# CartoonSegmentation/CartoonSegmentation

Measured on AMD Instinct MI355X. Metric: frames/sec at 1024x1024 (seg+depth+warp), higher is better.
Workload: dtype f32; 1 GPU; seg(RTMDet-Ins-L det640 + maskhead + ISNet refine@720, 2 instances) + LeReS depth@640 + 1 warp, frame 1024x1024; frames_per_gpu_step=8, global_batch=8, weights=closed-form synthetic (no checkpoints offline), precision=fp32 exact (v_mfma_f32_32x32x2_f32)

## Files before the change

cartoonsegmentation_amd/csrc/csm_convcfg.h:

```cpp
#pragma once
#include "csm_conv.h"
#include <span>
#include <utility>

#ifndef CSM_ILV
#define CSM_ILV 1
#endif

#ifdef CSM_CONV_ABLATE
#define CSM_DBG(a) ((a).dbg)
#else
#define CSM_DBG(a) 0
#endif

namespace csmconv {

constexpr int kLdsLd = 36;

typedef float f32x4v __attribute__((ext_vector_type(4)));

enum { CFG_128x128_4w = 0, CFG_128x64 = 1, CFG_64x64 = 2, CFG_128x128_8w = 3, CFG_128x32 = 4, CFG_64x16 = 5,
       CFG_D64x64 = 6, CFG_D128x64 = 7, CFG_D128x128 = 8, CFG_D128x128_8w = 9, CFG_D256x128_8w = 10, CFG_D64x128 = 11, CFG_D128x32 = 12,
       CFG_NARROW = 13,
       CFG_D96x128 = 14, CFG_D160x128 = 15, CFG_D224x128 = 16, CFG_D192x128 = 17,
       CFG_P64x64 = 18, CFG_P128x64 = 19, CFG_P64x128 = 20, CFG_P128x128 = 21, CFG_P256x128 = 22, CFG_P128x32 = 23,
       CFG_P64x64_w8 = 24, CFG_P128x128_w8 = 25, CFG_P128x32_w8 = 26, CFG_P128x128_8w = 27,
       CFG_D64x64_s3 = 28, CFG_D128x64_s3 = 29, CFG_D64x128_s3 = 30, CFG_D128x128_s3 = 31, CFG_D128x128_8w_s3 = 32,
       CFG_D256x128_8w_s3 = 33, CFG_D256x64 = 34, CFG_D256x64_s3 = 35, CFG_P256x64 = 36, CFG_D64x64_s4 = 37,
       CFG_Q64x64 = 38, CFG_Q128x64 = 39, CFG_Q64x128 = 40, CFG_Q128x128_8w = 41, CFG_Q128x32 = 42,
       CFG_R128x32 = 43, CFG_R64x64 = 44, CFG_R128x64 = 45, CFG_R128x32_w8 = 46, CFG_R128x128_8w = 47, CFG_R64x128 = 48, CFG_R64x64_w8 = 49,
       CFG_R128x128_8w_o4 = 50,
       CFG_W256x32 = 51, CFG_W256x64 = 52,
       CFG_COUNT = 53 };

enum ConvFamily {
    FAM_MFMA,
    FAM_DMA,
    FAM_PATCH,
    FAM_DMA_P,
    FAM_PATCH_P,
    FAM_WS,
    FAM_NARROW,
    FAM_COUNT
};
constexpr bool fam_uses_dma(int f) { return f != FAM_MFMA && f != FAM_NARROW; }
constexpr bool fam_needs_patch(int f) { return f == FAM_PATCH || f == FAM_PATCH_P || f == FAM_WS; }
constexpr bool fam_persistent(int f) { return f == FAM_DMA_P || f == FAM_PATCH_P || f == FAM_WS; }

struct ConvCfg {
    int id;
    const char *name;
    int family;
    int bn;
    int (*launch)(const ConvArgs &, hipStream_t);
};
std::span<const ConvCfg> conv_cfgs_mfma();
std::span<const ConvCfg> conv_cfgs_dma();
std::span<const ConvCfg> conv_cfgs_patch();
std::span<const ConvCfg> conv_cfgs_narrow();

bool dma_eligible(const ConvArgs &a);
bool patch_eligible(const ConvArgs &a);
bool narrow_eligible(const ConvArgs &a);
constexpr int kWsPatchBytes = 2 * (((16 + 2) * (16 + 2) + 7) / 8 + 1) * 1024;
bool ws_fits(const ConvArgs &a, int BN);

extern int g_ngroup_enable;
int choose_ngroup(const ConvArgs &a, int BN);
int launch_reduce(const ConvArgs &a, hipStream_t st);

int launch_conv_stem(const ConvArgs &a, hipStream_t st);
int launch_netop(const csm_op &op, int i, const View &in, const View &in1, const View &out, const float *weights, hipStream_t st);

}
```

cartoonsegmentation_amd/csrc/netops.hip:

```cpp
#include "csm_convcfg.h"

using namespace csmconv;

namespace {

__global__ __launch_bounds__(256) void k_conv_stem(ConvArgs a) {
    constexpr int BM = 64, BN = 64;
    __shared__ __attribute__((aligned(16))) float lds[(BM + BN) * kLdsLd];
    const int tid = threadIdx.x, lane = tid & 63, wave = tid >> 6;
    const int wm = wave >> 1, wn = wave & 1, li = lane & 31, lh = lane >> 5;
    int mt, ntile, zz;
    block_to_tile(mt, ntile, zz);
    const int m0 = mt * BM, n0 = ntile * BN;
    const int ho = a.out.h, wo = a.out.w, ntaps = a.kh * a.kw, nck = (ntaps + 7) >> 3;
    const int j = tid & 7;
    const float *rowp[2]; int iy0[2], ix0[2]; bool rv[2];
#pragma unroll
    for (int it = 0; it < 2; ++it) {
        int m = m0 + (tid >> 3) + 32 * it;
        rv[it] = m < a.M;
        int mm = rv[it] ? m : 0;
        int n = mm / (ho * wo), rem = mm - n * ho * wo;
        int oy = rem / wo, ox = rem - oy * wo;
        iy0[it] = oy * a.stride - a.pad; ix0[it] = ox * a.stride - a.pad;
// ... 319 lines not shown
    int b = blockIdx.x;
    const int tx = b % tiles_x; b /= tiles_x;
    const int ty = b % tiles_y, n = b / tiles_y;
    const int c0 = blockIdx.y * 32;
    const int oy0 = ty * TH, ox0 = tx * TW, iy0 = oy0 - a.pad, ix0 = ox0 - a.pad;
    for (int i = tid; i < taps * 32; i += 256) wl[i] = a.w[(int64_t)(i >> 5) * a.out.c + c0 + (i & 31)];
    const int total = rh * rw * 8;
    for (int i0 = tid; i0 < total; i0 += 256 * 4) {
        float4 v[4];
#pragma unroll
        for (int u = 0; u < 4; ++u) {
            int i = i0 + u * 256;
            v[u] = make_float4(0.f, 0.f, 0.f, 0.f);
            if (i < total) {
                int c4 = i & 7, pix = i >> 3;
                int ry = pix / rw, rx = pix - ry * rw;
                int iy = iy0 + ry, ix = ix0 + rx;
                if (iy >= 0 && iy < a.in.h && ix >= 0 && ix < a.in.w)
                    v[u] = *reinterpret_cast<const float4 *>(a.in.p + ((int64_t)(n * a.in.h + iy) * a.in.w + ix) * a.in.ld + c0 + c4 * 4);
            }
        }
#pragma unroll
        for (int u = 0; u < 4; ++u) {
            int i = i0 + u * 256;
            if (i < total) *reinterpret_cast<float4 *>(xl + (i >> 3) * 32 + (i & 7) * 4) = v[u];
        }
    }
    __syncthreads();
    const int c4 = tid & 7, p0 = tid >> 3;
    const float4 bias = a.bias ? *reinterpret_cast<const float4 *>(a.bias + c0 + c4 * 4) : make_float4(0.f, 0.f, 0.f, 0.f);
    const float4 sl = a.slope ? *reinterpret_cast<const float4 *>(a.slope + c0 + c4 * 4) : make_float4(0.f, 0.f, 0.f, 0.f);
    float4 acc[4];
#pragma unroll
    for (int j = 0; j < 4; ++j) acc[j] = bias;
    for (int kh = 0; kh < a.kh; ++kh)
        for (int kw = 0; kw < a.kw; ++kw) {
            const float4 w = *reinterpret_cast<const float4 *>(wl + (kh * a.kw + kw) * 32 + c4 * 4);
#pragma unroll
            for (int j = 0; j < 4; ++j) {
                const int pix = p0 + 32 * j, py = pix >> 4, px = pix & 15;
                const float4 x = *reinterpret_cast<const float4 *>(xl + ((py + kh) * rw + px + kw) * 32 + c4 * 4);
                acc[j].x = fmaf(x.x, w.x, acc[j].x); acc[j].y = fmaf(x.y, w.y, acc[j].y);
                acc[j].z = fmaf(x.z, w.z, acc[j].z); acc[j].w = fmaf(x.w, w.w, acc[j].w);
            }
        }
#pragma unroll
    for (int j = 0; j < 4; ++j) {
        const int pix = p0 + 32 * j, oy = oy0 + (pix >> 4), ox = ox0 + (pix & 15);
        if (oy >= a.out.h || ox >= a.out.w) continue;
        float4 v = acc[j];
        v.x = apply_act(v.x, a.act, sl.x); v.y = apply_act(v.y, a.act, sl.y);
        v.z = apply_act(v.z, a.act, sl.z); v.w = apply_act(v.w, a.act, sl.w);
        *reinterpret_cast<float4 *>(a.out.p + ((int64_t)(n * a.out.h + oy) * a.out.w + ox) * a.out.ld + c0 + c4 * 4) = v;
    }
}

__global__ __launch_bounds__(256) void k_maxpool(View in, View out, int k, int stride, int pad) {
    const int c4n = out.c >> 2;
    int64_t idx = (int64_t)blockIdx.x * 256 + threadIdx.x;
    int64_t total = (int64_t)out.n * out.h * out.w * c4n;
    if (idx >= total) return;
    int c = (int)(idx % c4n) * 4; int64_t pix = idx / c4n;
    int ox = (int)(pix % out.w); int64_t t = pix / out.w; int oy = (int)(t % out.h); int n = (int)(t / out.h);
    float4 m = make_float4(-INFINITY, -INFINITY, -INFINITY, -INFINITY);
    for (int ky = 0; ky < k; ++ky) {
        int iy = oy * stride - pad + ky;
        if (iy < 0 || iy >= in.h) continue;
        for (int kx = 0; kx < k; ++kx) {
            int ix = ox * stride - pad + kx;
            if (ix < 0 || ix >= in.w) continue;
            float4 x = *reinterpret_cast<const float4 *>(in.p + ((int64_t)(n * in.h + iy) * in.w + ix) * in.ld + c);
            m.x = fmaxf(m.x, x.x); m.y = fmaxf(m.y, x.y); m.z = fmaxf(m.z, x.z); m.w = fmaxf(m.w, x.w);
        }
    }
    *reinterpret_cast<float4 *>(out.p + pix * out.ld + c) = m;
}

__device__ __forceinline__ void src_index(int dst, int in_size, int out_size, float scale, bool align, int &i0, int &i1,
                                          float &l0, float &l1) {
    if (in_size == out_size) { i0 = i1 = dst; l0 = 1.0f; l1 = 0.0f; return; }
    float real;
    if (align) real = scale * (float)dst;
    else { real = scale * ((float)dst + 0.5f) - 0.5f; if (real < 0.0f) real = 0.0f; }
    i0 = min((int)real, in_size - 1);
    i1 = i0 + (i0 < in_size - 1 ? 1 : 0);
    l1 = fminf(fmaxf(real - (float)i0, 0.0f), 1.0f);
    l0 = 1.0f - l1;
}

template <int VEC>
__global__ __launch_bounds__(256) void k_bilinear(View in, View out, int align, float sh, float sw, int act, const float *__restrict__ slope) {
    const int cv = out.c / VEC;
    int64_t idx = (int64_t)blockIdx.x * 256 + threadIdx.x;
    int64_t total = (int64_t)out.n * out.h * out.w * cv;
    if (idx >= total) return;
    int c = (int)(idx % cv) * VEC; int64_t pix = idx / cv;
    int ox = (int)(pix % out.w); int64_t t = pix / out.w; int oy = (int)(t % out.h); int n = (int)(t / out.h);
    int y0, y1, x0, x1; float hl0, hl1, wl0, wl1;
    src_index(oy, in.h, out.h, sh, align != 0, y0, y1, hl0, hl1);
    src_index(ox, in.w, out.w, sw, align != 0, x0, x1, wl0, wl1);
    const float *P = in.p + (int64_t)n * in.h * in.w * in.ld + c;
    const float *a00 = P + ((int64_t)y0 * in.w + x0) * in.ld, *a01 = P + ((int64_t)y0 * in.w + x1) * in.ld;
    const float *a10 = P + ((int64_t)y1 * in.w + x0) * in.ld, *a11 = P + ((int64_t)y1 * in.w + x1) * in.ld;
    float *O = out.p + pix * out.ld + c;
    if (VEC == 4) {
        float4 p00 = *reinterpret_cast<const float4 *>(a00), p01 = *reinterpret_cast<const float4 *>(a01);
// ... 138 lines not shown
    for (int k = 0; k < K; ++k) {
        const float y = (lb[k] + (float)k * lx + (float)(K - 1 - k) * lo) / t;
        const float e = csm_expf(y - mx);
        den += e; num += e * c[k];
    }
    out.p[pix * out.ld] = num / den;
}

__global__ __launch_bounds__(256) void k_gavgpool(View in, View out) {
    __shared__ float part[256];
    int c = blockIdx.x, n = blockIdx.y;
    int hw = in.h * in.w;
    const float *P = in.p + (int64_t)n * hw * in.ld + c;
    float s = 0.0f;
    for (int i = threadIdx.x; i < hw; i += 256) s += P[(int64_t)i * in.ld];
    part[threadIdx.x] = s;
    __syncthreads();
    for (int st = 128; st >= 1; st >>= 1) {
        if ((int)threadIdx.x < st) part[threadIdx.x] += part[threadIdx.x + st];
        __syncthreads();
    }
    if (threadIdx.x == 0) out.p[(int64_t)n * out.ld + c] = part[0] / (float)hw;
}

__global__ __launch_bounds__(256) void k_gavgpool32(View in, View out) {
    __shared__ float part[256][33];
    const int c0 = blockIdx.x * 32, n = blockIdx.y, t = threadIdx.x;
    const int hw = in.h * in.w;
    const float *P = in.p + (int64_t)n * hw * in.ld + c0;
    float s[32];
#pragma unroll
    for (int c = 0; c < 32; ++c) s[c] = 0.0f;
    for (int i = t; i < hw; i += 256) {
        const float4 *q = reinterpret_cast<const float4 *>(P + (int64_t)i * in.ld);
#pragma unroll
        for (int c4 = 0; c4 < 8; ++c4) {
            float4 v = q[c4];
            s[4 * c4] += v.x; s[4 * c4 + 1] += v.y; s[4 * c4 + 2] += v.z; s[4 * c4 + 3] += v.w;
        }
    }
#pragma unroll
    for (int c = 0; c < 32; ++c) part[t][c] = s[c];
    __syncthreads();
    for (int st = 128; st >= 1; st >>= 1) {
        for (int i = t; i < st * 32; i += 256) {
            int r = i >> 5, c = i & 31;
            part[r][c] += part[r + st][c];
        }
        __syncthreads();
    }
    if (t < 32) out.p[(int64_t)n * out.ld + c0 + t] = part[0][t] / (float)hw;
}

__global__ __launch_bounds__(256) void k_nchw_to_nhwc(const float *__restrict__ src, int csrc, View out) {
    int64_t idx = (int64_t)blockIdx.x * 256 + threadIdx.x;
    int64_t total = (int64_t)out.n * out.h * out.w * out.c;
    if (idx >= total) return;
    int c = (int)(idx % out.c); int64_t pix = idx / out.c;
    int64_t hw = (int64_t)out.h * out.w; int64_t n = pix / hw, p = pix - n * hw;
    out.p[pix * out.ld + c] = c < csrc ? src[(n * csrc + c) * hw + p] : 0.0f;
}

__global__ __launch_bounds__(256) void k_nhwc_to_nchw(View in, float *__restrict__ dst) {
    int64_t idx = (int64_t)blockIdx.x * 256 + threadIdx.x;
    int64_t hw = (int64_t)in.h * in.w;
    int64_t total = (int64_t)in.n * in.c * hw;
    if (idx >= total) return;
    int64_t p = idx % hw; int64_t t = idx / hw; int c = (int)(t % in.c); int64_t n = t / in.c;
    dst[idx] = in.p[(n * hw + p) * in.ld + c];
}

constexpr int kTrPix = 64;
__global__ __launch_bounds__(256) void k_nchw_to_nhwc_tile(const float *__restrict__ src, int csrc, View out) {
    extern __shared__ float tr[];
    const int64_t hw = (int64_t)out.h * out.w;
    const int64_t tiles = (hw + kTrPix - 1) / kTrPix;
    const int64_t n = blockIdx.x / tiles, p0 = (blockIdx.x - n * tiles) * kTrPix;
    const int C = out.c;
    for (int i = threadIdx.x; i < C * kTrPix; i += 256) {
        const int c = i >> 6, p = i & 63;
        tr[c * (kTrPix + 1) + p] = (c < csrc && p0 + p < hw) ? src[(n * csrc + c) * hw + p0 + p] : 0.0f;
    }
    __syncthreads();
    for (int i = threadIdx.x; i < C * kTrPix; i += 256) {
        const int p = i / C, c = i - p * C;
        if (p0 + p < hw) out.p[(n * hw + p0 + p) * out.ld + c] = tr[c * (kTrPix + 1) + p];
    }
}
__global__ __launch_bounds__(256) void k_nhwc_to_nchw_tile(View in, float *__restrict__ dst) {
    extern __shared__ float tr[];
    const int64_t hw = (int64_t)in.h * in.w;
    const int64_t tiles = (hw + kTrPix - 1) / kTrPix;
    const int64_t n = blockIdx.x / tiles, p0 = (blockIdx.x - n * tiles) * kTrPix;
    const int C = in.c;
    for (int i = threadIdx.x; i < C * kTrPix; i += 256) {
        const int p = i / C, c = i - p * C;
        tr[c * (kTrPix + 1) + p] = p0 + p < hw ? in.p[(n * hw + p0 + p) * in.ld + c] : 0.0f;
    }
    __syncthreads();
    for (int i = threadIdx.x; i < C * kTrPix; i += 256) {
        const int c = i >> 6, p = i & 63;
        if (p0 + p < hw) dst[(n * C + c) * hw + p0 + p] = tr[c * (kTrPix + 1) + p];
    }
}

inline unsigned blocks_for(int64_t total) { return (unsigned)((total + 255) / 256); }

constexpr ConvCfg kRows[] = {{CFG_NARROW, "NARROW", FAM_NARROW, 4, &launch_narrow}};

}

std::span<const ConvCfg> csmconv::conv_cfgs_narrow() { return kRows; }

bool csmconv::narrow_eligible(const ConvArgs &a) {
    return a.cout_g <= 4 && a.groups == 1 && a.ksplit == 1 && !(a.cin_g & 3) && !(a.in.ld & 3) && narrow_lds(a, 4, nullptr, nullptr) != 0;
}

int csmconv::launch_reduce(const ConvArgs &a, hipStream_t st) {
    k_splitk_reduce<<<(unsigned)(((int64_t)a.M * a.cout_g + 255) / 256), 256, 0, st>>>(a);
    return csm::check_launch("k_splitk_reduce");
}

int csmconv::launch_conv_stem(const ConvArgs &a, hipStream_t st) {
    dim3 grid((a.M + 63) / 64, (a.cout_g + 63) / 64, 1);
    k_conv_stem<<<grid, 256, 0, st>>>(a);
    return csm::check_launch("k_conv_stem");
}

int csmconv::launch_netop(const csm_op &op, int i, const View &in, const View &in1, const View &out, const float *weights, hipStream_t st) {
    switch (op.kind) {
        case CSM_OP_DWCONV: {
            if ((in.ld & 3) || (out.ld & 3) || (out.c & 3)) { csm::set_error("op %d: dwconv needs c%%4==0", i); return CSM_ERR_ARG; }
            DwArgs a{in, out, weights + op.w_off, op.b_off >= 0 ? weights + op.b_off : nullptr,
                     op.aux_off >= 0 ? weights + op.aux_off : nullptr, op.kh, op.kw, op.stride, op.pad, op.dil, op.act};
            size_t lds = ((size_t)op.kh * op.kw * 32 + (size_t)(8 + op.kh - 1) * (16 + op.kw - 1) * 32) * 4;
            if (op.stride == 1 && op.dil == 1 && !(out.c & 31) && lds <= 64 * 1024 && out.h == in.h + 2 * op.pad - op.kh + 1) {
                int tiles_x = (out.w + 15) / 16, tiles_y = (out.h + 7) / 8;
                k_dwconv_lds<<<dim3((unsigned)(tiles_x * tiles_y * out.n), (unsigned)(out.c / 32)), 256, lds, st>>>(a, tiles_x, tiles_y);
            } else
                k_dwconv<<<blocks_for((int64_t)out.n * out.h * out.w * (out.c >> 2)), 256, 0, st>>>(a);
            break;
        }
        case CSM_OP_MAXPOOL:
            if ((in.ld & 3) || (out.ld & 3) || (out.c & 3)) { csm::set_error("op %d: maxpool needs c%%4==0", i); return CSM_ERR_ARG; }
            k_maxpool<<<blocks_for((int64_t)out.n * out.h * out.w * (out.c >> 2)), 256, 0, st>>>(in, out, op.kh, op.stride, op.pad);
            break;
        case CSM_OP_BILINEAR: {
            bool align = op.flags & 1;
            float sh, sw;
            if (align) { sh = out.h > 1 ? (float)(in.h - 1) / (float)(out.h - 1) : 0.0f; sw = out.w > 1 ? (float)(in.w - 1) / (float)(out.w - 1) : 0.0f; }
            else { sh = (float)in.h / (float)out.h; sw = (float)in.w / (float)out.w; }
            bool vec = !(out.c & 3) && !(in.ld & 3) && !(out.ld & 3) && !(((uintptr_t)in.p | (uintptr_t)out.p) & 15);
            const float *bsl = op.aux_off >= 0 ? weights + op.aux_off : nullptr;
            if (vec && out.h <= 65535 && out.n <= 65535 && (int64_t)out.w * (out.c >> 2) < (1ll << 30)) {
                unsigned mul, shr;
                set_fast_div((unsigned)(out.c >> 2), mul, shr);
                k_bilinear_rows<<<dim3(blocks_for((int64_t)out.w * (out.c >> 2)), (unsigned)out.h, (unsigned)out.n), 256, 0, st>>>(in, out, align ? 1 : 0, sh, sw, op.act, bsl, mul, shr);
            } else if (vec) k_bilinear<4><<<blocks_for((int64_t)out.n * out.h * out.w * (out.c >> 2)), 256, 0, st>>>(in, out, align ? 1 : 0, sh, sw, op.act, bsl);
            else k_bilinear<1><<<blocks_for((int64_t)out.n * out.h * out.w * out.c), 256, 0, st>>>(in, out, align ? 1 : 0, sh, sw, op.act, bsl);
            break;
        }
        case CSM_OP_NEAREST:
            if ((in.ld & 3) || (out.ld & 3) || (out.c & 3)) { csm::set_error("op %d: nearest needs c%%4==0", i); return CSM_ERR_ARG; }
            k_nearest<<<blocks_for((int64_t)out.n * out.h * out.w * (out.c >> 2)), 256, 0, st>>>(in, out);
            break;
        case CSM_OP_ADD:
            if (in.h < out.h || in.w < out.w || in.h > out.h + 1 || in.w > out.w + 1 || in1.h != out.h || in1.w != out.w) {
                csm::set_error("op %d: add: the first operand may exceed the output by at most one row / column", i); return CSM_ERR_ARG;
            }
            if (in.h == out.h && in.w == out.w && eltwise4_ok(in, &in1, out, nullptr))
                k_eltwise4<<<blocks_for((int64_t)out.n * out.h * out.w * (out.c >> 2)), 256, 0, st>>>(in, in1, out, op.act, 1, nullptr);
            else
                k_eltwise<<<blocks_for((int64_t)out.n * out.h * out.w * out.c), 256, 0, st>>>(in, in1, out, op.act,
                                                                                            (in.h != out.h || in.w != out.w) ? 3 : 1, nullptr);
            break;
        case CSM_OP_SCALE:
            k_eltwise<<<blocks_for((int64_t)out.n * out.h * out.w * out.c), 256, 0, st>>>(in, in1, out, op.act, 2, nullptr);
            break;
        case CSM_OP_ACT:
        case CSM_OP_COPY:
            if (eltwise4_ok(in, nullptr, out, op.aux_off >= 0 ? weights + op.aux_off : nullptr))
                k_eltwise4<<<blocks_for((int64_t)out.n * out.h * out.w * (out.c >> 2)), 256, 0, st>>>(in, in1, out, op.kind == CSM_OP_ACT ? op.act : 0, 0,
                                                                                                    op.aux_off >= 0 ? weights + op.aux_off : nullptr);
            else
                k_eltwise<<<blocks_for((int64_t)out.n * out.h * out.w * out.c), 256, 0, st>>>(in, in1, out, op.kind == CSM_OP_ACT ? op.act : 0, 0,
                                                                                              op.aux_off >= 0 ? weights + op.aux_off : nullptr);
            break;
        case CSM_OP_GAVGPOOL:
            if (!(in.c & 31) && !(in.ld & 3) && !(((uintptr_t)in.p) & 15)) k_gavgpool32<<<dim3(in.c / 32, in.n), 256, 0, st>>>(in, out);
            else k_gavgpool<<<dim3(in.c, in.n), 256, 0, st>>>(in, out);
            break;
        case CSM_OP_ATTRACTOR:
            if (op.aux_off < 0 || in.n != in1.n || in.h != in1.h || in.w != in1.w) { csm::set_error("op %d: attractor operands", i); return CSM_ERR_ARG; }
            k_attractor<<<blocks_for((int64_t)out.n * out.h * out.w * out.c), 256, 0, st>>>(in, in1, out, weights + op.aux_off, op.flags);
            break;
        case CSM_OP_LOGBINOM:
            if (op.aux_off < 0 || in.c < 4 || in1.c > 256) { csm::set_error("op %d: logbinom operands", i); return CSM_ERR_ARG; }
            k_logbinom<<<blocks_for((int64_t)out.n * out.h * out.w), 256, 0, st>>>(in, in1, out, weights + op.aux_off);
            break;
        case CSM_OP_NCHW_TO_NHWC:
            if (out.c >= 8 && out.c <= 240)
                k_nchw_to_nhwc_tile<<<(unsigned)(out.n * (((int64_t)out.h * out.w + kTrPix - 1) / kTrPix)), 256,
                                      sizeof(float) * (size_t)out.c * (kTrPix + 1), st>>>(in.p, in.c, out);
            else
                k_nchw_to_nhwc<<<blocks_for((int64_t)out.n * out.h * out.w * out.c), 256, 0, st>>>(in.p, in.c, out);
            break;
        case CSM_OP_NHWC_TO_NCHW:
            if (in.c >= 8 && in.c <= 240)
                k_nhwc_to_nchw_tile<<<(unsigned)(in.n * (((int64_t)in.h * in.w + kTrPix - 1) / kTrPix)), 256,
                                      sizeof(float) * (size_t)in.c * (kTrPix + 1), st>>>(in, out.p);
            else
                k_nhwc_to_nchw<<<blocks_for((int64_t)in.n * in.h * in.w * in.c), 256, 0, st>>>(in, out.p);
            break;
        default:
            csm::set_error("op %d: unknown kind %d", i, op.kind);
            return CSM_ERR_ARG;
    }
    return CSM_OK;
}
```

cartoonsegmentation_amd/csrc/nets.hip:

```cpp
#include "csm_common.h"
#include "csm_convcfg.h"
#include "csm_tokens.h"
#include <array>
#include <cstdio>
#include <cstdlib>
#include <cstring>
#include <map>
#include <mutex>
#include <vector>
#include <algorithm>
#include <utility>

using namespace csmconv;

int csmconv::g_ngroup_enable = 1;

static const ConvCfg &cfg_row(int id) {
    static const ConvCfg *table[CFG_COUNT];
    static const bool checked = [] {
        for (const std::span<const ConvCfg> rows : {conv_cfgs_mfma(), conv_cfgs_dma(), conv_cfgs_patch(), conv_cfgs_narrow()})
            for (const ConvCfg &r : rows) {
                if (r.id < 0 || r.id >= CFG_COUNT || table[r.id]) { fprintf(stderr, "csm355: conv tile configuration %d (%s) is out of range or defined twice\n", r.id, r.name); abort(); }
                table[r.id] = &r;
            }
// ... 118 lines not shown
                if (op.flags & CSM_CONV_FLAG_GROUPED) {
                    if (!grouped_eligible(a)) { csm::set_error("op %d: grouped-conv flag on an ineligible convolution (3x3 / stride 1 / pad 1 / cin_g == cout_g in {8, 16, 32} / channels %% 32 / ksplit 1)", i); return CSM_ERR_ARG; }
                    rc = launch_conv_grouped(a, st);
                    if (rc) return rc;
                    break;
                }
                if (op.flags & 2) {
                    if (op.groups != 1 || op.cin_g != 4 || a.ksplit != 1) { csm::set_error("op %d: stem flag needs groups 1, cin 4, ksplit 1", i); return CSM_ERR_ARG; }
                    rc = launch_conv_stem(a, st);
                    if (rc) return rc;
                    break;
                }
                const int tcfg = op.tile & (kTileSerial - 1);
                a.split = (op.tile & kTileSplit) != 0 && g_force_cfg < 0;
                const bool tuned = tcfg > 0 && tcfg <= CFG_COUNT && g_force_cfg < 0;
                a.serial = a.ksplit > 1 && (g_force_serial >= 0 ? g_force_serial != 0 : tuned ? (op.tile & kTileSerial) != 0
                                            : (int64_t)((a.M + 63) / 64) * ((op.cout_g + 63) / 64) >= 512);
                int cfg = tuned ? tcfg - 1 : choose_cfg(a, op.cout_g);
                rc = cfg_row(resolve_cfg(cfg, a)).launch(a, st);
                if (rc) return rc;
                break;
            }
            case CSM_OP_LAYERNORM: {
                if (op.w_off < 0 || op.b_off < 0 || op.aux_off < 0 || in.c != out.c) { csm::set_error("op %d: layernorm operands", i); return CSM_ERR_ARG; }
                rc = csm::launch_layernorm(in.p, in.ld, out.p, out.ld, (int64_t)in.n * in.h * in.w, in.c, weights + op.w_off, weights + op.b_off,
                                           weights + op.aux_off , st);
                if (rc) return rc;
                break;
            }
            case CSM_OP_ATTENTION: {
                const int heads = op.groups, d = op.cin_g;
                if (heads < 1 || in.c != 3 * heads * d || out.c != heads * d || in.w != 1 || out.h != in.h) { csm::set_error("op %d: attention operands", i); return CSM_ERR_ARG; }
                rc = csm::launch_attention(in.p, in.ld, out.p, out.ld, in.n, in.h, heads, d, op.aux_off >= 0 ? weights + op.aux_off : nullptr, op.kh, op.kw, st);
                if (rc) return rc;
                break;
            }
            case CSM_OP_TOKENS: {
                const int mode = op.flags;
                const int np = mode == 0 ? in.h * in.w : out.h * out.w;
                const bool ok = mode == 0 ? (out.h == np + 1 && out.w == 1 && out.c == in.c && op.aux_off >= 0)
                                          : (in.h == np + 1 && in.w == 1 && out.c == (mode == 1 ? 2 : 1) * in.c);
                if (!ok || in.n != out.n) { csm::set_error("op %d: tokens operands (mode %d)", i, mode); return CSM_ERR_ARG; }
                rc = csm::launch_tokens(mode, in.p, in.ld, out.p, out.ld, in.n, np, in.c, op.aux_off >= 0 ? weights + op.aux_off : nullptr, st);
                if (rc) return rc;
                break;
            }
            case CSM_OP_DEPTH_TO_SPACE: {
                const int k = op.stride;
                if (k < 1 || out.h != in.h * k || out.w != in.w * k || in.c != k * k * out.c) { csm::set_error("op %d: depth_to_space operands", i); return CSM_ERR_ARG; }
                rc = csm::launch_depth_to_space(in.p, in.ld, out.p, out.ld, in.n, in.h, in.w, k, out.c, st);
                if (rc) return rc;
                break;
            }
            default:
                rc = launch_netop(op, i, in, in1, out, weights, st);
                if (rc) return rc;
                break;
        }
        rc = csm::check_launch("program op");
        if (rc) { csm::set_error("op %d (kind %d) launch failed", i, op.kind); return rc; }
        if (ev) CSM_HIP(hipEventRecord(ev[i + 1], st));
    }
    return CSM_OK;
}

extern "C" int csm_run_program(const csm_op *ops, int n_ops, const csm_tensor_desc *tensors, int n_tensors,
                               const float *weights, float *workspace, void *const *ext, int n_ext, void *stream) {
    CSM_REQUIRE(ops && tensors && n_ops >= 0 && n_tensors > 0);
    return run_ops(ops, n_ops, tensors, n_tensors, weights, workspace, ext, n_ext, (hipStream_t)stream, nullptr);
}

struct EventSet {
    std::vector<hipEvent_t> ev;
    bool ok = true;
    explicit EventSet(size_t n) {
        ev.reserve(n);
        for (size_t i = 0; i < n; ++i) {
            hipEvent_t e;
            hipError_t r = hipEventCreate(&e);
            if (r != hipSuccess) { csm::set_error("hipEventCreate: %s", hipGetErrorString(r)); ok = false; return; }
            ev.push_back(e);
        }
    }
    ~EventSet() { for (auto e : ev) (void)hipEventDestroy(e); }
    EventSet(const EventSet &) = delete;
    EventSet &operator=(const EventSet &) = delete;
};

extern "C" int csm_run_program_profile(const csm_op *ops, int n_ops, const csm_tensor_desc *tensors, int n_tensors,
                                       const float *weights, float *workspace, void *const *ext, int n_ext, void *stream,
                                       float *op_ms) {
    CSM_REQUIRE(ops && tensors && op_ms && n_ops >= 0 && n_tensors > 0);
    hipStream_t st = (hipStream_t)stream;
    EventSet evs(n_ops + 1);
    if (!evs.ok) return CSM_ERR_HIP;
    int rc = run_ops(ops, n_ops, tensors, n_tensors, weights, workspace, ext, n_ext, st, evs.ev.data());
    if (rc == CSM_OK) {
        hipError_t e = hipStreamSynchronize(st);
        if (e != hipSuccess) { csm::set_error("profile sync: %s", hipGetErrorString(e)); rc = CSM_ERR_HIP; }
        else for (int i = 0; i < n_ops; ++i) (void)hipEventElapsedTime(&op_ms[i], evs.ev[i], evs.ev[i + 1]);
    }
    return rc;
}

static std::map<std::array<int, 16>, int> g_tile_cache;
static std::mutex g_tile_mutex;

extern "C" int csm_conv_autotune(csm_op *ops, int n_ops, const csm_tensor_desc *tensors, int n_tensors, const float *weights,
                                 float *workspace, void *const *ext, int n_ext, void *stream, int reps) {
    CSM_REQUIRE(ops && tensors && n_ops >= 0 && n_tensors > 0);
// ... 83 lines not shown
            if (timed[k].first < best) { best = timed[k].first; best_cfg = timed[k].second; }
        if (rc) break;
        op.tile = best_cfg >= 0 ? best_cfg + 1 : 0;
        { std::lock_guard<std::mutex> lk(g_tile_mutex); g_tile_cache[key] = op.tile; }
        ++tuned;
    }
    return rc == CSM_OK ? tuned : -rc;
}

extern "C" int csm_conv_tile_cache_save(const char *path) {
    CSM_REQUIRE(path);
    FILE *f = fopen(path, "w");
    if (!f) { csm::set_error("cannot write %s", path); return CSM_ERR_ARG; }
    std::lock_guard<std::mutex> lk(g_tile_mutex);
    for (const auto &kv : g_tile_cache) {
        for (int v : kv.first) fprintf(f, "%d ", v);
        fprintf(f, "%d\n", kv.second);
    }
    fclose(f);
    return CSM_OK;
}

extern "C" int csm_conv_tile_cache_load(const char *path) {
    CSM_REQUIRE(path);
    FILE *f = fopen(path, "r");
    if (!f) return 0;
    int n = 0;
    for (;;) {
        std::array<int, 16> key; int tile = 0; bool ok = true;
        for (int &v : key) ok = ok && fscanf(f, "%d", &v) == 1;
        if (!ok || fscanf(f, "%d", &tile) != 1) break;
        if (tile >= 0 && (tile & (kTileSerial - 1)) <= CFG_COUNT && tile < 2 * kTileSplit) { std::lock_guard<std::mutex> lk(g_tile_mutex); g_tile_cache[key] = tile; ++n; }
    }
    fclose(f);
    return n;
}

extern "C" int csm_debug_force_conv_cfg(int cfg) {
    if (cfg >= 0) { g_force_cfg = cfg & 0xff; g_dbg = cfg >> 8; } else { g_force_cfg = -1; g_dbg = 0; }
    return CSM_OK;
}

extern "C" int csm_debug_conv_tuner_options(int options) {
    g_tune_split = options & 1;
    g_ngroup_enable = (options & 2) ? 0 : 1;
    return CSM_OK;
}

extern "C" int csm_debug_force_splitk_serial(int mode) {
    g_force_serial = mode < 0 ? -1 : (mode ? 1 : 0);
    return CSM_OK;
}

extern "C" int csm_debug_conv_cfg_count(void) { return CFG_COUNT; }

extern "C" int csm_debug_conv_cfg_info(int cfg, csm_conv_cfg_desc *info) {
    CSM_REQUIRE(info);
    if (cfg < 0 || cfg >= CFG_COUNT) { csm::set_error("conv tile configuration %d out of range (0 .. %d)", cfg, CFG_COUNT - 1); return CSM_ERR_ARG; }
    static const char *const fam_names[FAM_COUNT] = {"MFMA", "DMA", "PATCH", "DMA_P", "PATCH_P", "WS", "NARROW"};
    const ConvCfg &r = cfg_row(cfg);
    info->id = r.id; info->bn = r.bn; info->name = r.name; info->family = fam_names[r.family];
    info->tune_pos = -1;
    for (size_t k = 0; k < sizeof(kTuneOrder) / sizeof(int); ++k)
        if (kTuneOrder[k] == cfg) info->tune_pos = (int)k;
    return CSM_OK;
}

extern "C" int csm_debug_conv_resolve_cfg(int cfg, const csm_op *op, const csm_tensor_desc *in_desc, const csm_tensor_desc *out_desc) {
    if (!op || !in_desc || !out_desc || cfg < 0 || cfg >= CFG_COUNT) { csm::set_error("conv_resolve_cfg: bad argument"); return -CSM_ERR_ARG; }
    return resolve_cfg(cfg, conv_args(*op, view_at(nullptr, *in_desc), view_at(nullptr, *out_desc), View{}, nullptr));
}
```

cartoonsegmentation_amd/program.py:

```python
import ctypes
import os

import numpy as np

OP_CONV, OP_DWCONV, OP_MAXPOOL, OP_BILINEAR, OP_NEAREST, OP_ADD, OP_GAVGPOOL, OP_SCALE = 1, 2, 3, 4, 5, 6, 7, 8
OP_NCHW_TO_NHWC, OP_NHWC_TO_NCHW, OP_ACT, OP_COPY, OP_ATTRACTOR, OP_LOGBINOM = 9, 10, 11, 12, 13, 14
OP_LAYERNORM, OP_ATTENTION, OP_TOKENS, OP_DEPTH_TO_SPACE = 15, 16, 17, 18
ACT = {None: 0, 'none': 0, 'relu': 1, 'silu': 2, 'prelu': 3, 'hsigmoid': 4, 'sigmoid': 5, 'softplus': 6, 'gelu': 7}


class CsmTensorDesc(ctypes.Structure):
    _fields_ = [("offset", ctypes.c_int64), ("ext", ctypes.c_int32), ("n", ctypes.c_int32), ("h", ctypes.c_int32),
                ("w", ctypes.c_int32), ("c", ctypes.c_int32), ("ld", ctypes.c_int32)]


class CsmOp(ctypes.Structure):
    _fields_ = [("kind", ctypes.c_int32), ("in0", ctypes.c_int32), ("in1", ctypes.c_int32), ("out", ctypes.c_int32),
                ("kh", ctypes.c_int32), ("kw", ctypes.c_int32), ("stride", ctypes.c_int32), ("pad", ctypes.c_int32),
                ("dil", ctypes.c_int32), ("groups", ctypes.c_int32), ("cin_g", ctypes.c_int32),
                ("cout_g", ctypes.c_int32), ("act", ctypes.c_int32), ("res_mode", ctypes.c_int32),
                ("w_off", ctypes.c_int64), ("b_off", ctypes.c_int64), ("aux_off", ctypes.c_int64),
                ("flags", ctypes.c_int32), ("ksplit", ctypes.c_int32), ("scratch", ctypes.c_int32),
                ("tile", ctypes.c_int32)]

# ... 388 lines not shown
        w_h, w_n = self._w(gamma, gamma)
        b_h, b_n = self._w(beta, beta)
        a_h, a_n = self._w(np.array([eps, 0, 0, 0], np.float32), np.array([eps, 0, 0, 0], np.float32))
        return self._emit(OP_LAYERNORM, x, None, out, w_off=w_h, b_off=b_h, aux_off=a_h, nat=dict(w_off=w_n, b_off=b_n, aux_off=a_n))

    def attention(self, qkv, heads, grid=None, rel_table=None):
        d = qkv.c // (3 * heads)
        assert qkv.w == 1 and qkv.c == 3 * heads * d and d in (32, 64, 128), (qkv.shape, heads)
        out = self.buffer(qkv.n, qkv.h, 1, heads * d)
        a_h = a_n = -1
        gh, gw = grid if grid is not None else (0, 0)
        if rel_table is not None:
            rel_table = np.asarray(rel_table, np.float32)
            assert rel_table.shape == ((2 * gh - 1) * (2 * gw - 1) + 3, heads) and qkv.h == gh * gw + 1, (rel_table.shape, grid, qkv.h)
            a_h, a_n = self._w(np.ascontiguousarray(rel_table.T), rel_table)
        self.flops += 4 * qkv.n * heads * qkv.h * qkv.h * d
        self.flops_exec += 4 * qkv.n * heads * qkv.h * qkv.h * d
        return self._emit(OP_ATTENTION, qkv, None, out, groups=heads, cin_g=d, kh=gh, kw=gw, aux_off=a_h, nat=dict(aux_off=a_n))

    def tokens_assemble(self, patches, cls):
        out = self.buffer(patches.n, patches.h * patches.w + 1, 1, patches.c)
        a_h, a_n = self._w(cls, cls)
        return self._emit(OP_TOKENS, patches, None, out, flags=0, aux_off=a_h, nat=dict(aux_off=a_n))

    def tokens_readout(self, tokens, grid, project=True):
        gh, gw = grid
        assert tokens.w == 1 and tokens.h == gh * gw + 1
        out = self.buffer(tokens.n, gh, gw, tokens.c * (2 if project else 1))
        return self._emit(OP_TOKENS, tokens, None, out, flags=1 if project else 2, kh=gh, kw=gw)

    def depth_to_space(self, x, k):
        assert x.c % (k * k) == 0 and (x.c // (k * k)) % 4 == 0
        out = self.buffer(x.n, x.h * k, x.w * k, x.c // (k * k))
        return self._emit(OP_DEPTH_TO_SPACE, x, None, out, stride=k)

    def conv_transpose_nonoverlap(self, x, w, b, k):
        w = np.asarray(w, np.float32)
        cin, cout = w.shape[0], w.shape[1]
        assert w.shape[2:] == (k, k) and cin == x.c
        w1 = w.transpose(2, 3, 1, 0).reshape(k * k * cout, cin, 1, 1)
        b1 = None if b is None else np.tile(np.asarray(b, np.float32), k * k)
        return self.depth_to_space(self.conv(x, w1, b1), k)

    def crop_rows(self, x, h):
        assert x.n == 1 and 0 < h <= x.h and x.coff == 0 and x.c == x.buf.c
        b = Buf(1, h, x.w, x.buf.c)
        b.alias = x.buf
        b.first, b.last = x.buf.first, x.buf.last
        self.bufs.append(b)
        return T(self, b, 0, x.c)

    def gavgpool(self, x):
        out = self.buffer(x.n, 1, 1, x.c)
        return self._emit(OP_GAVGPOOL, x, None, out)

    def scale(self, x, s, out=None):
        if out is None:
            out = self.buffer(x.n, x.h, x.w, x.c)
        return self._emit(OP_SCALE, x, s, out)

    def keep(self, t):
        t.buf.keep = True
        return t

    def plan(self):
        ALIGN = 64
        free, top = [], 0
        by_first, by_last = {}, {}
        for b in self.bufs:
            if b.ext >= 0 or b.first is None or b.alias is not None:
                continue
            b.size = (b.n * b.h * b.w * b.c + ALIGN - 1) // ALIGN * ALIGN
            by_first.setdefault(b.first, []).append(b)
            if not b.keep:
                by_last.setdefault(b.last, []).append(b)
        for i in range(len(self.ops)):
            for b in by_first.get(i, []):
                best = None
                for k, (off, sz) in enumerate(free):
                    if sz >= b.size and (best is None or sz < free[best][1]):
                        best = k
                if best is None:
                    b.offset = top; top += b.size
                else:
                    off, sz = free.pop(best)
                    b.offset = off
                    if sz > b.size:
                        free.append((off + b.size, sz - b.size))
            for b in by_last.get(i, []):
                free.append((b.offset, b.size))
                free.sort()
                merged = []
                for off, sz in free:
                    if merged and merged[-1][0] + merged[-1][1] == off:
                        merged[-1] = (merged[-1][0], merged[-1][1] + sz)
                    else:
                        merged.append((off, sz))
                free = merged
        for b in self.bufs:
            if b.alias is not None:
                b.offset = b.alias.offset
        self.workspace_floats = top
        return top

    def serialise(self, oracle=False):
        if getattr(self, "workspace_floats", None) is None:
            self.plan()
# ... 18 lines not shown
```

include/csm355.h:

```cpp
#ifndef CSM355_H
#define CSM355_H
#include <stddef.h>
#include <stdint.h>
#ifdef __cplusplus
extern "C" {
#endif

#define CSM_OK 0
#define CSM_ERR_ARG 1
#define CSM_ERR_HIP 2
#define CSM_ERR_NAN 3
#define CSM_ERR_DATA 4

const char *csm_last_error(void);
int csm_version(void);
const char *csm_build_info(void);


int csm_pointrender_update_zee(const float *pts, int B, int64_t N, int H, int W, double focal,
                               double baseline, float *zee, void *stream);

int csm_pointrender_degrid(const float *zee_in, float *zee_out, int B, int H, int W, void *stream);

int csm_pointrender_update_output(const float *pts, const float *data, const float *zee, int B, int C,
// ... 61 lines not shown
    CSM_OP_GAVGPOOL = 7,
    CSM_OP_SCALE = 8,
    CSM_OP_NCHW_TO_NHWC = 9,
    CSM_OP_NHWC_TO_NCHW = 10,
    CSM_OP_ACT = 11,
    CSM_OP_COPY = 12,
    CSM_OP_ATTRACTOR = 13,
    CSM_OP_LOGBINOM = 14,
    CSM_OP_LAYERNORM = 15,
    CSM_OP_ATTENTION = 16,
    CSM_OP_TOKENS = 17,
    CSM_OP_DEPTH_TO_SPACE = 18
};
enum csm_act { CSM_ACT_NONE = 0, CSM_ACT_RELU = 1, CSM_ACT_SILU = 2, CSM_ACT_PRELU = 3, CSM_ACT_HSIGMOID = 4,
               CSM_ACT_SIGMOID = 5, CSM_ACT_SOFTPLUS = 6 ,
               CSM_ACT_GELU = 7  };

typedef struct csm_tensor_desc {
    int64_t offset;
    int32_t ext;
    int32_t n, h, w, c;
    int32_t ld;
} csm_tensor_desc;

#define CSM_CONV_FLAG_STEM 2
#define CSM_CONV_FLAG_WINOGRAD 4
#define CSM_CONV_FLAG_WINOGRAD4 8
#define CSM_CONV_FLAG_GROUPED 16

typedef struct csm_op {
    int32_t kind;
    int32_t in0, in1, out;
    int32_t kh, kw, stride, pad, dil;
    int32_t groups;
    int32_t cin_g, cout_g;
    int32_t act, res_mode;
    int64_t w_off, b_off, aux_off;
    int32_t flags;
    int32_t ksplit;
    int32_t scratch;
    int32_t tile;
} csm_op;

int csm_conv_autotune(csm_op *ops, int n_ops, const csm_tensor_desc *tensors, int n_tensors, const float *weights,
                      float *workspace, void *const *ext, int n_ext, void *stream, int reps);

int csm_conv_tile_cache_save(const char *path);
int csm_conv_tile_cache_load(const char *path);

int csm_run_program(const csm_op *ops, int n_ops, const csm_tensor_desc *tensors, int n_tensors,
                    const float *weights, float *workspace, void *const *ext, int n_ext, void *stream);
int csm_debug_force_conv_cfg(int cfg);
int csm_debug_force_splitk_serial(int mode);
int csm_debug_conv_tuner_options(int options);
typedef struct csm_conv_cfg_desc {
    int32_t id;
    int32_t bn;
    int32_t tune_pos;
    const char *name;
    const char *family;
} csm_conv_cfg_desc;
int csm_debug_conv_cfg_count(void);
int csm_debug_conv_cfg_info(int cfg, csm_conv_cfg_desc *info);
int csm_debug_conv_resolve_cfg(int cfg, const csm_op *op, const csm_tensor_desc *in_desc, const csm_tensor_desc *out_desc);
int csm_debug_attention_options(int options);
int csm_run_program_profile(const csm_op *ops, int n_ops, const csm_tensor_desc *tensors, int n_tensors,
                            const float *weights, float *workspace, void *const *ext, int n_ext, void *stream,
                            float *op_ms);


size_t csm_mean_std_scratch_bytes(void);
int csm_mean_std(const float *x, int64_t n, float *out2, void *scratch, void *stream);
int csm_normalise_mean_std(const float *x, int64_t n, const float *mean_std_dev, float *out, void *stream);
int csm_denormalise_mean_std(const float *x, int64_t n, const float *mean_std_dev, int mode, float *out, void *stream);
int csm_resize_bilinear_planes(const float *in, int planes, int H, int W, int h, int w, int align_corners, float *out, void *stream);
int csm_mask_area_resize_threshold(const uint8_t *masks, int n, int H, int W, int h, int w, float thr, uint8_t *out, void *stream);


int csm_zoe_pad_prep(const float *img, int B, int H, int W, int pad_h, int pad_w, int flip, int nh, int nw, float *out, void *stream);
int csm_zoe_resize_crop(const float *d, int B, int h, int w, int pad_h, int pad_w, int H, int W, int unflip, int mode, float *out,
                        void *stream);
int csm_zoe_depth_to_disparity(const float *depth, int64_t n, float focal_times_baseline, float *out, void *stream);


int csm_pack_mask_bits(const uint8_t *mask, int64_t n, uint8_t *out, void *stream);

int csm_det_decode_slots(const int *level_hw, int n_levels, int num_classes, int nms_pre);
size_t csm_det_decode_scratch_bytes(int nb, int slots);
int csm_det_decode(const float *const *cls, const float *const *reg, const int *level_hw, const int *strides, const int *lds3,
                   int n_levels, int nb, int num_classes, float score_thr, int nms_pre, float clamp_w, float clamp_h,
                   float scale_x, float scale_y, float min_bbox_size, int K, float *scores, float *boxes, int *src, int *labels,
                   float *class_offsets, void *scratch, void *stream);
int csm_det_gather(const float *const *kern, const int *level_hw, const int *strides, const int *lds3, int n_levels, int nb, int K,
                   int max_keep, int num_gen_params, const int *keep, const float *scores, const float *boxes, const int *src,
                   const int *labels, float *kept_scores, float *kept_boxes, int *kept_labels, float *kept_priors,
                   float *kept_kernels, void *stream);

size_t csm_nms_scratch_bytes(int n);
int csm_nms(const float *boxes, const float *class_offsets, int n, float iou_thr, int max_keep, int *keep,
            int *n_keep, void *scratch, void *stream);
size_t csm_nms_batch_scratch_bytes(int nb, int n);
int csm_nms_batch(const float *boxes, const float *class_offsets, int nb, int n, float iou_thr, int max_keep, int *keep,
                  int *n_keep, void *scratch, void *stream);

int csm_maskhead_logits(const float *mask_feat, int ld, int h, int w, int num_prototypes, int dyconv_channels,
                        const float *kernels, const float *priors, int n, int feat_stride, float *logits,
// ... 161 lines not shown
```

Before: 138.0 frames/s.

## Add column-walk 5x5 depthwise conv, split global avgpool, and vectorized scale kernel

Adds a register-resident sliding-window 5x5 depthwise conv kernel. Each thread walks down a column of 4 channels and reuses loaded input rows across the K output rows via a rotating accumulator. It also splits global average pooling into a wide partials pass plus a tree reduction using a new scratch buffer, so large spatial inputs get more parallelism. A float4 broadcast-scale kernel replaces the generic eltwise path. Debug knobs select the forms, and the program builder now allocates gavgpool scratch.

Measured after the change: 138.4 frames/s, median of 4. About the same (+0.3%).

```diff
diff --git a/cartoonsegmentation_amd/csrc/csm_convcfg.h b/cartoonsegmentation_amd/csrc/csm_convcfg.h
--- a/cartoonsegmentation_amd/csrc/csm_convcfg.h
+++ b/cartoonsegmentation_amd/csrc/csm_convcfg.h
@@ -70,6 +70,7 @@
 int launch_reduce(const ConvArgs &a, hipStream_t st);
 
 int launch_conv_stem(const ConvArgs &a, hipStream_t st);
-int launch_netop(const csm_op &op, int i, const View &in, const View &in1, const View &out, const float *weights, hipStream_t st);
+int launch_netop(const csm_op &op, int i, const View &in, const View &in1, const View &out, const View &scratch, const float *weights, hipStream_t st);
+int set_netop_form(int kind, int form);
 
 }
diff --git a/cartoonsegmentation_amd/csrc/netops.hip b/cartoonsegmentation_amd/csrc/netops.hip
--- a/cartoonsegmentation_amd/csrc/netops.hip
+++ b/cartoonsegmentation_amd/csrc/netops.hip
@@ -395,6 +395,73 @@
         v.x = apply_act(v.x, a.act, sl.x); v.y = apply_act(v.y, a.act, sl.y);
         v.z = apply_act(v.z, a.act, sl.z); v.w = apply_act(v.w, a.act, sl.w);
         *reinterpret_cast<float4 *>(a.out.p + ((int64_t)(n * a.out.h + oy) * a.out.w + ox) * a.out.ld + c0 + c4 * 4) = v;
+    }
+}
+
+template <int K, int ACT>
+__global__ __launch_bounds__(256) void k_dwconv_col(DwArgs a, int rows_per, unsigned c4_mul, unsigned c4_shr) {
+    const int act = ACT >= 0 ? ACT : a.act;
+    const int c4n = a.out.c >> 2, j = blockIdx.x * 256 + threadIdx.x;
+    if (j >= a.out.w * c4n) return;
+    const int ox = (int)fast_div((unsigned)j, c4_mul, c4_shr), c = (j - ox * c4n) * 4;
+    const int n = blockIdx.z, oy0 = blockIdx.y * rows_per, rows = min(rows_per, a.out.h - oy0);
+    const int steps = rows + K - 1, iy0 = oy0 - a.pad, ix0 = ox - a.pad;
+    float4 w[K * K];
+#pragma unroll
+    for (int t = 0; t < K * K; ++t) w[t] = *reinterpret_cast<const float4 *>(a.w + (int64_t)t * a.out.c + c);
+    float4 bias = make_float4(0.f, 0.f, 0.f, 0.f), sl = make_float4(0.f, 0.f, 0.f, 0.f);
+    if (a.bias) bias = *reinterpret_cast<const float4 *>(a.bias + c);
+    if (a.slope) sl = *reinterpret_cast<const float4 *>(a.slope + c);
+    const float *base = a.in.p + (int64_t)n * a.in.h * a.in.w * a.in.ld + c;
+    float *orow = a.out.p + (((int64_t)n * a.out.h + oy0 - (K - 1)) * a.out.w + ox) * a.out.ld + c;
+    const int64_t ostep = (int64_t)a.out.w * a.out.ld;
+    int coff[K]; bool colv[K];
+#pragma unroll
+    for (int kw = 0; kw < K; ++kw) {
+        colv[kw] = ix0 + kw >= 0 && ix0 + kw < a.in.w;
+        coff[kw] = min(max(ix0 + kw, 0), a.in.w - 1) * a.in.ld;
+    }
+    auto load_row = [&](int i, float4 (&x)[K]) {
+        const int iy = iy0 + i;
+        const float *rp = base + (int64_t)min(max(iy, 0), a.in.h - 1) * a.in.w * a.in.ld;
+#pragma unroll
+        for (int kw = 0; kw < K; ++kw) x[kw] = *reinterpret_cast<const float4 *>(rp + coff[kw]);
+    };
+    float4 acc[K];
+#pragma unroll
+    for (int s = 0; s < K; ++s) acc[s] = bias;
+    auto step = [&](int i, float4 (&x)[K]) {
+        const int iy = iy0 + i;
+        const bool rv = iy >= 0 && iy < a.in.h;
+#pragma unroll
+        for (int kw = 0; kw < K; ++kw)
+            if (!(rv && colv[kw])) x[kw] = make_float4(0.f, 0.f, 0.f, 0.f);
+#pragma unroll
+        for (int kh = K - 1; kh >= 0; --kh) {
+            float4 v = kh == 0 ? bias : acc[kh - 1];
+#pragma unroll
+            for (int kw = 0; kw < K; ++kw) {
+                const float4 ww = w[kh * K + kw];
+                v.x = fmaf(x[kw].x, ww.x, v.x); v.y = fmaf(x[kw].y, ww.y, v.y);
+                v.z = fmaf(x[kw].z, ww.z, v.z); v.w = fmaf(x[kw].w, ww.w, v.w);
+            }
+            acc[kh] = v;
+        }
+        if (i >= K - 1) {
+            float4 v = acc[K - 1];
+            v.x = apply_act(v.x, act, sl.x); v.y = apply_act(v.y, act, sl.y);
+            v.z = apply_act(v.z, act, sl.z); v.w = apply_act(v.w, act, sl.w);
+            *reinterpret_cast<float4 *>(orow + i * ostep) = v;
+        }
+    };
+    float4 xa[K], xb[K];
+    load_row(0, xa);
+    for (int i = 0; i < steps; i += 2) {
+        load_row(i + 1, xb);
+        step(i, xa);
+        if (i + 1 >= steps) break;
+        load_row(i + 2, xa);
+        step(i + 1, xb);
     }
 }
 
@@ -639,6 +706,54 @@
     if (t < 32) out.p[(int64_t)n * out.ld + c0 + t] = part[0][t] / (float)hw;
 }
 
+__global__ __launch_bounds__(256) void k_gavgpool_partials(View in, float *__restrict__ part, unsigned c4_mul, unsigned c4_shr) {
+    const int c4n = in.c >> 2, j = blockIdx.x * 256 + threadIdx.x;
+    const int t = (int)fast_div((unsigned)j, c4_mul, c4_shr), c = (j - t * c4n) * 4, n = blockIdx.y;
+    const int hw = in.h * in.w;
+    const float *P = in.p + (int64_t)n * hw * in.ld + c;
+    float4 s = make_float4(0.f, 0.f, 0.f, 0.f);
+    int i = t;
+    for (; i + 7 * 256 < hw; i += 8 * 256) {
+        float4 v[8];
+#pragma unroll
+        for (int u = 0; u < 8; ++u) v[u] = *reinterpret_cast<const float4 *>(P + (int64_t)(i + u * 256) * in.ld);
+#pragma unroll
+        for (int u = 0; u < 8; ++u) { s.x += v[u].x; s.y += v[u].y; s.z += v[u].z; s.w += v[u].w; }
+    }
+    for (; i < hw; i += 256) {
+        const float4 v = *reinterpret_cast<const float4 *>(P + (int64_t)i * in.ld);
+        s.x += v.x; s.y += v.y; s.z += v.z; s.w += v.w;
+    }
+    *reinterpret_cast<float4 *>(part + ((int64_t)n * 256 + t) * in.c + c) = s;
+}
+__global__ __launch_bounds__(256) void k_gavgpool_tree(const float *__restrict__ partials, View in, View out) {
+    __shared__ float part[256][33];
+    const int c0 = blockIdx.x * 32, n = blockIdx.y, t = threadIdx.x;
+    for (int i = t; i < 256 * 32; i += 256) part[i >> 5][i & 31] = partials[((int64_t)n * 256 + (i >> 5)) * in.c + c0 + (i & 31)];
+    __syncthreads();
+    for (int st = 128; st >= 1; st >>= 1) {
+        for (int i = t; i < st * 32; i += 256) {
+            int r = i >> 5, c = i & 31;
+            part[r][c] += part[r + st][c];
+        }
+        __syncthreads();
+    }
+    if (t < 32) out.p[(int64_t)n * out.ld + c0 + t] = part[0][t] / (float)(in.h * in.w);
+}
+
+__global__ __launch_bounds__(256) void k_scale4(View a, View b, View out, int act, unsigned c4_mul, unsigned c4_shr) {
+    const int c4n = out.c >> 2, j = blockIdx.x * 256 + threadIdx.x, n = blockIdx.y;
+    const int hw = out.h * out.w;
+    if (j >= hw * c4n) return;
+    const int p = (int)fast_div((unsigned)j, c4_mul, c4_shr), c = (j - p * c4n) * 4;
+    const int64_t pix = (int64_t)n * hw + p;
+    float4 v = *reinterpret_cast<const float4 *>(a.p + pix * a.ld + c);
+    const float4 w = *reinterpret_cast<const float4 *>(b.p + (int64_t)n * b.ld + c);
+    v.x = v.x * w.x; v.y = v.y * w.y; v.z = v.z * w.z; v.w = v.w * w.w;
+    v.x = apply_act(v.x, act, 0.0f); v.y = apply_act(v.y, act, 0.0f); v.z = apply_act(v.z, act, 0.0f); v.w = apply_act(v.w, act, 0.0f);
+    *reinterpret_cast<float4 *>(out.p + pix * out.ld + c) = v;
+}
+
 __global__ __launch_bounds__(256) void k_nchw_to_nhwc(const float *__restrict__ src, int csrc, View out) {
     int64_t idx = (int64_t)blockIdx.x * 256 + threadIdx.x;
     int64_t total = (int64_t)out.n * out.h * out.w * out.c;
@@ -693,6 +808,14 @@
 
 inline unsigned blocks_for(int64_t total) { return (unsigned)((total + 255) / 256); }
 
+int g_form_dwconv = -1, g_form_gavg = -1, g_form_scale = -1;
+
+int dwcol_rows(const View &out, int k) {
+    const int64_t col_blocks = (int64_t)blocks_for((int64_t)out.w * (out.c >> 2)) * out.n;
+    const int segs = (int)std::max<int64_t>(1, 512 / col_blocks);
+    return std::max(k - 1, (out.h + segs - 1) / segs);
+}
+
 constexpr ConvCfg kRows[] = {{CFG_NARROW, "NARROW", FAM_NARROW, 4, &launch_narrow}};
 
 }
@@ -714,14 +837,42 @@
     return csm::check_launch("k_conv_stem");
 }
 
-int csmconv::launch_netop(const csm_op &op, int i, const View &in, const View &in1, const View &out, const float *weights, hipStream_t st) {
+int csmconv::set_netop_form(int kind, int form) {
+    switch (kind) {
+        case CSM_OP_DWCONV: if (form < -1 || (form >= 0 && (form & 255) > 2)) break; g_form_dwconv = form; return CSM_OK;
+        case CSM_OP_GAVGPOOL: if (form < -1 || form > 2) break; g_form_gavg = form; return CSM_OK;
+        case CSM_OP_SCALE: if (form < -1 || form > 1) break; g_form_scale = form; return CSM_OK;
+        default: csm::set_error("csm_debug_netop_form: kind %d has one form", kind); return CSM_ERR_ARG;
+    }
+    csm::set_error("csm_debug_netop_form: kind %d has no form %d", kind, form);
+    return CSM_ERR_ARG;
+}
+
+int csmconv::launch_netop(const csm_op &op, int i, const View &in, const View &in1, const View &out, const View &scratch, const float *weights, hipStream_t st) {
     switch (op.kind) {
         case CSM_OP_DWCONV: {
             if ((in.ld & 3) || (out.ld & 3) || (out.c & 3)) { csm::set_error("op %d: dwconv needs c%%4==0", i); return CSM_ERR_ARG; }
             DwArgs a{in, out, weights + op.w_off, op.b_off >= 0 ? weights + op.b_off : nullptr,
                      op.aux_off >= 0 ? weights + op.aux_off : nullptr, op.kh, op.kw, op.stride, op.pad, op.dil, op.act};
             size_t lds = ((size_t)op.kh * op.kw * 32 + (size_t)(8 + op.kh - 1) * (16 + op.kw - 1) * 32) * 4;
-            if (op.stride == 1 && op.dil == 1 && !(out.c & 31) && lds <= 64 * 1024 && out.h == in.h + 2 * op.pad - op.kh + 1) {
+            const int form = g_form_dwconv < 0 ? -1 : (g_form_dwconv & 255);
+            const bool col_ok = op.kh == 5 && op.kw == 5 && op.stride == 1 && op.dil == 1 && out.h == in.h + 2 * op.pad - 4 && out.w == in.w + 2 * op.pad - 4 &&
+                                !(((uintptr_t)in.p | (uintptr_t)out.p | (uintptr_t)a.w | (uintptr_t)a.bias | (uintptr_t)a.slope) & 15) &&
+                                (int64_t)out.w * (out.c >> 2) < (1ll << 30) && out.n <= 65535;
+            if (form == 2 && !col_ok) { csm::set_error("op %d: dwconv form 2 (column walk) needs 5x5 / stride 1 / dilation 1 and 16-byte aligned views", i); return CSM_ERR_ARG; }
+            if (col_ok && (form == 2 || form < 0)) {
+                int rows = form == 2 && (g_form_dwconv >> 8) > 0 ? (g_form_dwconv >> 8) : dwcol_rows(out, 5);
+                rows = std::max(rows, (out.h + 65534) / 65535);
+                unsigned mul, shr;
+                set_fast_div((unsigned)(out.c >> 2), mul, shr);
+                const dim3 grid(blocks_for((int64_t)out.w * (out.c >> 2)), (unsigned)((out.h + rows - 1) / rows), (unsigned)out.n);
+                switch (op.act) {
+                    case CSM_ACT_NONE: k_dwconv_col<5, CSM_ACT_NONE><<<grid, 256, 0, st>>>(a, rows, mul, shr); break;
+                    case CSM_ACT_RELU: k_dwconv_col<5, CSM_ACT_RELU><<<grid, 256, 0, st>>>(a, rows, mul, shr); break;
+                    case CSM_ACT_SILU: k_dwconv_col<5, CSM_ACT_SILU><<<grid, 256, 0, st>>>(a, rows, mul, shr); break;
+                    default: k_dwconv_col<5, -1><<<grid, 256, 0, st>>>(a, rows, mul, shr); break;
+                }
+            } else if (form != 0 && op.stride == 1 && op.dil == 1 && !(out.c & 31) && lds <= 64 * 1024 && out.h == in.h + 2 * op.pad - op.kh + 1) {
                 int tiles_x = (out.w + 15) / 16, tiles_y = (out.h + 7) / 8;
                 k_dwconv_lds<<<dim3((unsigned)(tiles_x * tiles_y * out.n), (unsigned)(out.c / 32)), 256, lds, st>>>(a, tiles_x, tiles_y);
             } else
@@ -762,7 +913,12 @@
                                                                                             (in.h != out.h || in.w != out.w) ? 3 : 1, nullptr);
             break;
         case CSM_OP_SCALE:
-            k_eltwise<<<blocks_for((int64_t)out.n * out.h * out.w * out.c), 256, 0, st>>>(in, in1, out, op.act, 2, nullptr);
+            if (g_form_scale != 0 && eltwise4_ok(in, &in1, out, nullptr) && (int64_t)out.h * out.w * (out.c >> 2) < (1ll << 30) && out.n <= 65535) {
+                unsigned mul, shr;
+                set_fast_div((unsigned)(out.c >> 2), mul, shr);
+                k_scale4<<<dim3(blocks_for((int64_t)out.h * out.w * (out.c >> 2)), (unsigned)out.n), 256, 0, st>>>(in, in1, out, op.act, mul, shr);
+            } else
+                k_eltwise<<<blocks_for((int64_t)out.n * out.h * out.w * out.c), 256, 0, st>>>(in, in1, out, op.act, 2, nullptr);
             break;
         case CSM_OP_ACT:
         case CSM_OP_COPY:
@@ -773,10 +929,22 @@
                 k_eltwise<<<blocks_for((int64_t)out.n * out.h * out.w * out.c), 256, 0, st>>>(in, in1, out, op.kind == CSM_OP_ACT ? op.act : 0, 0,
                                                                                               op.aux_off >= 0 ? weights + op.aux_off : nullptr);
             break;
-        case CSM_OP_GAVGPOOL:
-            if (!(in.c & 31) && !(in.ld & 3) && !(((uintptr_t)in.p) & 15)) k_gavgpool32<<<dim3(in.c / 32, in.n), 256, 0, st>>>(in, out);
+        case CSM_OP_GAVGPOOL: {
+            const bool v32 = !(in.c & 31) && !(in.ld & 3) && !(((uintptr_t)in.p) & 15);
+            const bool split_ok = v32 && scratch.p && !(((uintptr_t)scratch.p) & 15) && scratch.ld == scratch.c &&
+                                  (int64_t)scratch.n * scratch.h * scratch.w * scratch.c >= (int64_t)in.n * 256 * in.c && in.n <= 65535;
+            if (g_form_gavg == 2 && !split_ok) { csm::set_error("op %d: gavgpool form 2 (split) needs c %% 32 == 0, a 16-byte aligned input and a scratch tensor of n * 256 * c floats", i); return CSM_ERR_ARG; }
+            if (split_ok && (g_form_gavg == 2 || (g_form_gavg < 0 && in.h * in.w >= 4096))) {
+                unsigned mul, shr;
+                set_fast_div((unsigned)(in.c >> 2), mul, shr);
+                k_gavgpool_partials<<<dim3((unsigned)(in.c >> 2), (unsigned)in.n), 256, 0, st>>>(in, scratch.p, mul, shr);
+                k_gavgpool_tree<<<dim3(in.c / 32, in.n), 256, 0, st>>>(scratch.p, in, out);
+                break;
+            }
+            if (v32 && g_form_gavg != 0) k_gavgpool32<<<dim3(in.c / 32, in.n), 256, 0, st>>>(in, out);
             else k_gavgpool<<<dim3(in.c, in.n), 256, 0, st>>>(in, out);
             break;
+        }
         case CSM_OP_ATTRACTOR:
             if (op.aux_off < 0 || in.n != in1.n || in.h != in1.h || in.w != in1.w) { csm::set_error("op %d: attractor operands", i); return CSM_ERR_ARG; }
             k_attractor<<<blocks_for((int64_t)out.n * out.h * out.w * out.c), 256, 0, st>>>(in, in1, out, weights + op.aux_off, op.flags);
diff --git a/cartoonsegmentation_amd/csrc/nets.hip b/cartoonsegmentation_amd/csrc/nets.hip
--- a/cartoonsegmentation_amd/csrc/nets.hip
+++ b/cartoonsegmentation_amd/csrc/nets.hip
@@ -194,10 +194,13 @@
                 if (rc) return rc;
                 break;
             }
-            default:
-                rc = launch_netop(op, i, in, in1, out, weights, st);
-                if (rc) return rc;
-                break;
+            default: {
+                View sc{};
+                if (op.scratch >= 0) { rc = make_view(tensors, n_tensors, op.scratch, workspace, ext, n_ext, sc); if (rc) return rc; }
+                rc = launch_netop(op, i, in, in1, out, sc, weights, st);
+                if (rc) return rc;
+                break;
+            }
         }
         rc = csm::check_launch("program op");
         if (rc) { csm::set_error("op %d (kind %d) launch failed", i, op.kind); return rc; }
@@ -387,6 +390,8 @@
     return CSM_OK;
 }
 
+extern "C" int csm_debug_netop_form(int kind, int form) { return set_netop_form(kind, form); }
+
 extern "C" int csm_debug_conv_cfg_count(void) { return CFG_COUNT; }
 
 extern "C" int csm_debug_conv_cfg_info(int cfg, csm_conv_cfg_desc *info) {
diff --git a/cartoonsegmentation_amd/program.py b/cartoonsegmentation_amd/program.py
--- a/cartoonsegmentation_amd/program.py
+++ b/cartoonsegmentation_amd/program.py
@@ -464,7 +464,10 @@
 
     def gavgpool(self, x):
         out = self.buffer(x.n, 1, 1, x.c)
-        return self._emit(OP_GAVGPOOL, x, None, out)
+        scr = None
+        if x.c % 32 == 0:
+            scr = self.buffer(x.n, 1, 256, x.c)
+        return self._emit(OP_GAVGPOOL, x, None, out, scratch=-1 if scr is None else scr.id, scratch_view=scr)
 
     def scale(self, x, s, out=None):
         if out is None:
diff --git a/include/csm355.h b/include/csm355.h
--- a/include/csm355.h
+++ b/include/csm355.h
@@ -137,6 +137,7 @@
                     const float *weights, float *workspace, void *const *ext, int n_ext, void *stream);
 int csm_debug_force_conv_cfg(int cfg);
 int csm_debug_force_splitk_serial(int mode);
+int csm_debug_netop_form(int kind, int form);
 int csm_debug_conv_tuner_options(int options);
 typedef struct csm_conv_cfg_desc {
     int32_t id;
```
